# lucanest/Phyloformer

Hardware: AMD Instinct MI355X
Metric: alignments/sec, 60-leaf/500-site LG+GC-like MSAs, Phyloformer forward (pf.ckpt) (higher is better)
Workload: dtype f16x3-split MFMA (two fp16 limbs per operand, 3 passes), fp32 accumulate/residual

## Files before the change

phyloformer_amd/csrc/pf_device.hip.h:

```cpp
#pragma once
#include <hip/hip_runtime.h>
#include <stdint.h>

#include "pf_layout.h"

namespace pfk {

typedef float f32x4 __attribute__((ext_vector_type(4)));
typedef float f32x16 __attribute__((ext_vector_type(16)));
#if PF_F16
typedef _Float16 h16_t;
#define PF_MFMA(a, b, c) __builtin_amdgcn_mfma_f32_32x32x16_f16((a), (b), (c), 0, 0, 0)
#define PF_DOT2C "v_dot2c_f32_f16"
#define PF_CVT_PK "v_cvt_pk_f16_f32"
#define PF_NEG1_LO 0x0000bc00u
#define PF_NEG1_HI 0xbc000000u
#else
typedef __bf16 h16_t;
#define PF_MFMA(a, b, c) __builtin_amdgcn_mfma_f32_32x32x16_bf16((a), (b), (c), 0, 0, 0)
#define PF_DOT2C "v_dot2c_f32_bf16"
#define PF_CVT_PK "v_cvt_pk_bf16_f32"
#define PF_NEG1_LO 0x0000bf80u
#define PF_NEG1_HI 0xbf800000u
#endif
// ... 289 lines not shown
    const frag_t* wv_lo;
    const float* table;
    const uint8_t* idx;
    const int16_t* pair_i;
    const int16_t* pair_j;
    int B, N, P, Lloc;
    int flat;
    int nt_aln;
    int slots_aln;
    size_t trash_tok;
    int store_x_last;
    unsigned long long* prof;
    int ablate;
    float* sitemap;
    const float* w;
};

enum { MODE_FIRST = 0, MODE_MID = 1, MODE_LAST = 2, MODE_MID0 = 3, MODE_LAST_FOLD = 4 };

struct TilePos { int b, kt, r0, l0; };
template <bool FLAT>
__device__ __forceinline__ TilePos tile_pos(const MainArgs& a, int task, int ntiles) {
    TilePos q;
    q.b = task / a.nt_aln;
    q.kt = task - q.b * a.nt_aln;
    if (FLAT) { const int tok0 = q.kt * 32; q.r0 = tok0 / a.Lloc; q.l0 = tok0 - q.r0 * a.Lloc; }
    else { q.r0 = q.kt / ntiles; q.l0 = (q.kt - q.r0 * ntiles) * 32; }
    return q;
}
template <bool FLAT>
__device__ __forceinline__ TilePos tile_next(const MainArgs& a, TilePos q) {
    if (++q.kt == a.nt_aln) { q.b++; q.kt = 0; q.r0 = 0; q.l0 = 0; return q; }
    q.l0 += 32;
// ... 2 lines not shown
}
struct LanePos { size_t tok0; int toff, l, nvalid, wrap; bool valid, in_r1; };
template <bool FLAT>
__device__ __forceinline__ LanePos lane_pos(const MainArgs& a, const TilePos& q, int t) {
    LanePos o;
    o.tok0 = ((size_t)q.b * a.P + q.r0) * a.Lloc + q.l0;
    const int left = FLAT ? a.P * a.Lloc - q.kt * 32 : a.Lloc - q.l0;
    o.nvalid = min(32, left);
    o.wrap = (FLAT && q.r0 + 1 < a.P) ? min(32, a.Lloc - q.l0) : 32;
    o.valid = t < o.nvalid;
    o.toff = min(t, o.nvalid - 1);
    o.in_r1 = o.toff >= o.wrap;
    o.l = q.l0 + o.toff - (o.in_r1 ? a.Lloc : 0);
    return o;
}
__device__ __forceinline__ void part_range(int flat, int pr, int nparts, int P, int L, int slots_aln, long* first, int* count) {
    if (!flat) { *first = (long)pr * nparts; *count = nparts; return; }
    const int b = pr / P, p = pr - b * P;
    const int k0 = (int)(((long)p * L) >> 5), k1 = (int)((((long)p + 1) * L - 1) >> 5);
    *first = (long)b * slots_aln + k0 + p;
    *count = k1 - k0 + 1;
}

template <int LO, int HI>
__device__ __forceinline__ void image_to_lds(const frag_t* src, unsigned char* smem) {
    static_assert(LO % 64 == 0 && HI % 64 == 0, "the image is copied in whole waves");
    const int wv = threadIdx.x >> 6, ln = threadIdx.x & 63;
#pragma unroll
    for (int k = 0; k < (HI - LO + MAIN_THREADS - 1) / MAIN_THREADS; ++k) {
        const int f0 = LO + k * MAIN_THREADS + wv * 64;
        if (f0 < HI) __builtin_amdgcn_global_load_lds(src + f0 + ln, smem + (size_t)f0 * 16, 16, 0, 0);
    }
}

template <int MODE, bool FLAT, bool SITEMAP = false, bool WEIGHTED = false>
__global__ void __launch_bounds__(MAIN_THREADS, MAIN_WAVES / 4) k_main(MainArgs a) {
    constexpr bool LAST = MODE == MODE_LAST || MODE == MODE_LAST_FOLD;
    constexpr bool FOLD = MODE == MODE_LAST_FOLD;
    static_assert(!SITEMAP || LAST, "the site map is the head's: last block only");
    static_assert(!WEIGHTED || (!SITEMAP && MODE != MODE_FIRST), "weighted launches: blocks' own modes, no site map");
    extern __shared__ __attribute__((aligned(16))) unsigned char smem[];
    lds_frag_t lw = (lds_frag_t)smem;
    lds_f32_t lc = (lds_f32_t)(smem + FRAG_END * 16);

    {
        const float cv = a.consts[min((int)threadIdx.x, CONST_LEN - 1)];
        if (FOLD) {
            image_to_lds<FRAG_W1, FRAG_W2>(a.wimg, smem);
            image_to_lds<FRAG_WO, FRAG_U + U_FRAGS>(a.wimg, smem);
        } else {
            image_to_lds<(MODE == MODE_FIRST) ? FRAG_WV : 0, LAST ? FRAG_WV : FRAG_END>(a.wimg, smem);
        }
        static_assert(CONST_LEN <= MAIN_THREADS, "one constant per thread");
// ... 23 lines not shown

    {
        const int nwaves = gridDim.x * MAIN_WAVES;
#ifndef PF_RUN_MAX
#define PF_RUN_MAX 8
#endif
        const int run = max(1, min(PF_RUN_MAX, ntasks / (nwaves * 8)));
        int run0 = (blockIdx.x * MAIN_WAVES + wave) * run;
        const int task0 = run0, task1 = ntasks;
        TilePos cur = tile_pos<FLAT>(a, min(task0, ntasks - 1), ntiles);
        int frag_row = -1;
        frag_t mfr[4];
        f32x4 rqv = {0.f, 0.f, 0.f, 0.f};
        f32x4 px[8], pctx[8], pqr, pqc;
        int pri = 0, prj = 0;
        auto prefetch = [&](const TilePos& np) {
            const LanePos nl = lane_pos<FLAT>(a, np, t);
            const int ll = nl.l, pb = np.b;
            const size_t tk = nl.tok0 + nl.toff;
            if (MODE == MODE_MID0) {
                const uint8_t* ib = a.idx + (size_t)pb * a.N * a.Lloc + ll;
                const int pp = np.r0 + (nl.in_r1 ? 1 : 0);
                pri = residue(ib[(size_t)a.pair_i[pp] * a.Lloc]);
                prj = residue(ib[(size_t)a.pair_j[pp] * a.Lloc]);
            } else {
                const f32x4* xp = reinterpret_cast<const f32x4*>(a.x + tk * 64 + 4 * h);
#pragma unroll
                for (int g = 0; g < 8; ++g) px[g] = xp[2 * g];
            }
            pqr = *reinterpret_cast<const f32x4*>(a.qrow + tk * 4);
            pqc = *reinterpret_cast<const f32x4*>(a.qcol + tk * 4);
            if (MODE != MODE_FIRST) {
                int hq = h;
                asm volatile("" : "+v"(hq));
                const f32x4* cp = reinterpret_cast<const f32x4*>(a.ctx + ((size_t)pb * a.Lloc + ll) * 64 + 4 * hq);
#pragma unroll
                for (int g = 0; g < 8; ++g) pctx[g] = cp[2 * g];
            }
        };
        if (MODE != MODE_FIRST && task0 < task1) prefetch(cur);

        for (int task = task0; task < task1;) {
            const int b = cur.b;
            const int row = b * a.P + cur.r0;
            int ntask = task + 1;
            TilePos nxt = tile_next<FLAT>(a, cur);
            if (ntask == run0 + run) {
                run0 += nwaves * run;
                ntask = run0;
                if (ntask < task1) nxt = tile_pos<FLAT>(a, ntask, ntiles);
            }
            const LanePos lp = lane_pos<FLAT>(a, cur, t);
            const bool straddle = lp.wrap < 32;
            int ai = 0, aj = 0;
            if (MODE == MODE_FIRST) { const int pp = cur.r0 + (lp.in_r1 ? 1 : 0); ai = a.pair_i[pp]; aj = a.pair_j[pp]; }
            auto load_mfr = [&](int r) {
                const frag_t* mf = a.mfrag + (size_t)r * 128 + t;
#pragma unroll
                for (int q = 0; q < 4; ++q) mfr[q] = mf[q * 32];
                typedef const f32x4 __attribute__((address_space(4)))* const_f32x4_t;
                rqv = *(const_f32x4_t)(unsigned long long)(a.rq + (size_t)__builtin_amdgcn_readfirstlane(r) * 4);
                frag_row = r;
            };
            if (MODE != MODE_FIRST && row != frag_row) load_mfr(row);
            const bool valid = lp.valid;
// ... 4 lines not shown
            float wt = 1.f;
            if (WEIGHTED && LAST) wt = a.w[(size_t)b * a.Lloc + lc_];

            if (MODE == MODE_FIRST) {
                const int ri = residue(a.idx[((size_t)b * a.N + ai) * a.Lloc + lc_]);
                const int rj = residue(a.idx[((size_t)b * a.N + aj) * a.Lloc + lc_]);
                const f32x4* ti = reinterpret_cast<const f32x4*>(a.table + ri * 64 + 4 * h);
                const f32x4* tj = reinterpret_cast<const f32x4*>(a.table + rj * 64 + 4 * h);
#pragma unroll
                for (int g = 0; g < 8; ++g) {
                    f32x4 u = ti[2 * g], w = tj[2 * g];
#pragma unroll
                    for (int i = 0; i < 4; ++i) x[4 * g + i] = u[i] + w[i];
                }
            } else {
                if (MODE == MODE_MID0) {
                    const f32x4* ti = reinterpret_cast<const f32x4*>(a.table + pri * 64 + 4 * h);
                    const f32x4* tj = reinterpret_cast<const f32x4*>(a.table + prj * 64 + 4 * h);
#pragma unroll
                    for (int g = 0; g < 8; ++g) {
                        const f32x4 u = ti[2 * g], w = tj[2 * g];
#pragma unroll
                        for (int i = 0; i < 4; ++i) x[4 * g + i] = u[i] + w[i];
                    }
                } else {
#pragma unroll
                    for (int g = 0; g < 8; ++g)
#pragma unroll
                        for (int i = 0; i < 4; ++i) x[4 * g + i] = px[g][i];
                }
                PF_TICK(0);
// ... 89 lines not shown
                    }
                    PF_TICK(3);
                } else if (!(a.ablate & 16)) {
                    frag_t xb_hi[4], xb_lo[4];
                    {
                        float xn[32];
                        ln_pair(x, xn);
#pragma unroll
                        for (int s = 0; s < 4; ++s) split8(&xn[8 * s], xb_hi[s], xb_lo[s]);
                    }
                    f32x16 oa[2];
                    load_acc_bias(oa[0], lch + CONST_B2);
                    load_acc_bias(oa[1], lch + CONST_B2 + 32);
#pragma unroll
                    for (int j = 0; j < 32; ++j) oa[j >> 4][j & 15] += x[j];
                    if (ntask < task1) prefetch(nxt);
                    PF_TICK(2);
#pragma unroll 1
                    for (int T = 0; T < 8; ++T) {
                        f32x16 ha;
                        lds_frag_t f1 = w1p + T * 512;
                        lds_frag_t f2 = w2p + T * 256;
                        lds_f32_t bp = lch + CONST_B1 + 32 * T;
                        PF_OPAQUE(f1); PF_OPAQUE(f2); PF_OPAQUE(bp);
                        load_acc_bias(ha, bp);
                        frag_t fh = f1[0], fl = f1[64];
#pragma unroll
                        for (int s = 0; s < 4; ++s) {
                            frag_t nh, nl;
                            if (s < 3) { nh = f1[(s + 1) * 128]; nl = f1[(s + 1) * 128 + 64]; }
                            else { nh = f2[0]; nl = f2[64]; }
// ... 218 lines not shown
                if (valid) {
                    if (WEIGHTED) {
                        acc += wl * s;
                        acce += wl * e;
                    } else {
                        acc += s;
                        acce += e;
                    }
                    const size_t tok = row0 + l;
                    if (a.x) {
                        const int ra = rr / 22, rb = rr - 22 * ra;
                        const f32x4 xa = *reinterpret_cast<const f32x4*>(emb + ra * 64 + 4 * cl);
                        const f32x4 xb = *reinterpret_cast<const f32x4*>(emb + rb * 64 + 4 * cl);
                        *reinterpret_cast<f32x4*>(a.x + tok * 64 + 4 * cl) = xa + xb;
                    }
                    if (cl == 0) *reinterpret_cast<f32x4*>(a.qrow + tok * 4) = e;
                }
            };
            if (lbase + 64 <= a.Lloc) {
#pragma unroll 4
                for (int it = 0; it < 16; ++it) site(it, true);
            } else {
                for (int it = 0; it < nit; ++it) site(it, lbase + 4 * it + sg < a.Lloc);
            }
            cur = nxt;
            wcur = wnxt;
        }
#pragma unroll
        for (int i = 0; i < 4; ++i) {
            acc[i] += __shfl_xor(acc[i], 16);
            acc[i] += __shfl_xor(acc[i], 32);
// ... 147 lines not shown
    const float* x;
    const float* qrow;
    const float* mrow;
    float* qcol;
    float* part;
    const float* wqk;
    const float* bqk;
    const float* brow;
    int B, P, Lloc, G, nchunks;
    int sub, S, fine;
    const float* table;
    const uint8_t* idx;
    const int16_t* pair_i;
    const int16_t* pair_j;
    int N;
};
constexpr int CPART = 4 * 64 + 8;

constexpr int CS_SLOT = 2 * 256 + 64;
#ifndef PF_CS_RING
#define PF_CS_RING 4
#endif
#ifndef PF_CS_MT
#define PF_CS_MT 16
#endif
template <bool EMBED, int RING, int MT>
#ifndef PF_CS_WAVES
#define PF_CS_WAVES 2
#endif
__global__ void __launch_bounds__(256, PF_CS_WAVES) k_colstats(ColStatsArgs a) {
    static_assert(!(EMBED && RING), "block 0 reads residue bytes, not x");
    static_assert(RING % 2 == 0, "pairs are consumed two at a time");
    static_assert(MT == 16 || MT == 8, "pair matrices are staged 16 or 8 at a time (runs are multiples of 8)");
    constexpr int LDS_MST = 2 * MT * MROW, LDS_RING = RING ? 4 * RING * CS_SLOT : 0, LDS_EMB = EMBED ? 22 * 64 : 0;
    constexpr int PIJ_CAP = 640;
    __shared__ __attribute__((aligned(16))) float lds_all[LDS_MST + LDS_RING + LDS_EMB + (EMBED ? PIJ_CAP : 0)];
    float* const mst = lds_all;
    float* const xring = lds_all + LDS_MST;
    float* const emb = lds_all + LDS_MST + LDS_RING;
    int16_t* const pij = reinterpret_cast<int16_t*>(lds_all + LDS_MST + LDS_RING + LDS_EMB);
    if (EMBED) {
        constexpr int NV = 22 * 64 / 4;
        const f32x4* tsrc = reinterpret_cast<const f32x4*>(a.table);
        const int i0 = threadIdx.x, i1 = threadIdx.x + 256;
        static_assert(NV <= 2 * 256, "two vectors per thread cover the table");
        const f32x4 v0 = tsrc[min(i0, NV - 1)], v1 = tsrc[min(i1, NV - 1)];
        if (i0 < NV) reinterpret_cast<f32x4*>(emb)[i0] = v0;
        if (i1 < NV) reinterpret_cast<f32x4*>(emb)[i1] = v1;
    }
    const int lane = threadIdx.x & 63, wave = threadIdx.x >> 6;
    const int ts = lane >> 3, cl = lane & 7;
    const int per = (a.P + a.G - 1) / a.G;

    f32x2 w2[4][8];
#pragma unroll
    for (int o = 0; o < 8; o += 2)
#pragma unroll
        for (int q = 0; q < 2; ++q) {
            const f32x4 u0 = *reinterpret_cast<const f32x4*>(a.wqk + o * 64 + 8 * cl + 4 * q);
            const f32x4 u1 = *reinterpret_cast<const f32x4*>(a.wqk + (o + 1) * 64 + 8 * cl + 4 * q);
#pragma unroll
            for (int i = 0; i < 4; ++i) w2[o >> 1][4 * q + i] = f32x2{u0[i], u1[i]};
        }
// ... 32 lines not shown

    f32x4 nx0[2], nx1[2], nqr[2];
    int nri[2] = {0, 0}, nrj[2] = {0, 0};
    const bool pij_lds = EMBED && (p1 - p0) <= PIJ_CAP;
    if (pij_lds) {
        for (int i = threadIdx.x; i < p1 - p0; i += 256) { pij[i] = a.pair_i[p0 + i]; pij[PIJ_CAP + i] = a.pair_j[p0 + i]; }
        __syncthreads();
    }
    auto fetch = [&](int p, int u) {
        const int pc = min(p, a.P - 1);
        const size_t tk = ((size_t)b * a.P + pc) * a.Lloc + lcl;
        if (!EMBED) {
            nx0[u] = *reinterpret_cast<const f32x4*>(a.x + tk * 64 + 8 * cl);
            nx1[u] = *reinterpret_cast<const f32x4*>(a.x + tk * 64 + 8 * cl + 4);
        }
        nqr[u] = *reinterpret_cast<const f32x4*>(a.qrow + tk * 4);
    };
    float* const wring = xring + (RING ? wave * RING * CS_SLOT : 0);
    const int lq = min(chunk * 32 + wave * 8 + ((lane & 31) >> 2), a.Lloc - 1);
    auto issue = [&](int p, size_t lane_off) {
        const int pc = min(p, a.P - 1);
        const size_t row = ((size_t)b * a.P + pc) * a.Lloc;
        float* dst = wring + ((p - p0) % RING) * CS_SLOT;
        const float* xs = a.x + row * 64 + lane_off;
        __builtin_amdgcn_global_load_lds(xs, dst, 16, 0, 0);
        __builtin_amdgcn_global_load_lds(xs + 4, dst + 256, 16, 0, 0);
        __builtin_amdgcn_global_load_lds(a.qrow + (row + lq) * 4 + (lane & 3), dst + 512, 4, 0, 0);
    };
    const size_t lane_off0 = (size_t)lcl * 64 + 8 * cl;
    auto take = [&](int p, int u) {
        const float* slot = wring + ((p - p0) % RING) * CS_SLOT;
// ... 3 lines not shown
    };
    auto fetch_idx = [&](int p, int u) {
        const int pc = min(p, a.P - 1);
        const uint8_t* ib = a.idx + (size_t)b * a.N * a.Lloc + lcl;
        const int pl = min(pc, p1 - 1) - p0;
        const int si = pij_lds ? (int)pij[pl] : (int)a.pair_i[pc];
        const int sj = pij_lds ? (int)pij[PIJ_CAP + pl] : (int)a.pair_j[pc];
        nri[u] = residue(ib[(size_t)si * a.Lloc]);
        nrj[u] = residue(ib[(size_t)sj * a.Lloc]);
    };
    auto lookup = [&](int u) {
        const float* ei = emb + nri[u] * 64 + 8 * cl;
        const float* ej = emb + nrj[u] * 64 + 8 * cl;
        nx0[u] = *reinterpret_cast<const f32x4*>(ei) + *reinterpret_cast<const f32x4*>(ej);
        nx1[u] = *reinterpret_cast<const f32x4*>(ei + 4) + *reinterpret_cast<const f32x4*>(ej + 4);
    };
    auto stage = [&](int pt, int buf) {
        const f32x4* src = reinterpret_cast<const f32x4*>(a.mrow + ((size_t)b * a.P + pt) * MROW);
        const int n4 = min(MT, p1 - pt) * (MROW / 4);
        float* dst = mst + (size_t)buf * MT * MROW;
#pragma unroll
        for (int k = 0; k < MT * MROW / 4 / 256; ++k) {
            const int i = (int)threadIdx.x + 256 * k;
            __builtin_amdgcn_global_load_lds(src + min(i, n4 - 1), dst + (256 * k + 64 * wave) * 4, 16, 0, 0);
        }
    };
    stage(p0, 0);
    if (RING) {
#pragma unroll
        for (int i = 0; i < RING; ++i) issue(p0 + i, lane_off0);
// ... 262 lines not shown
```

phyloformer_amd/csrc/pf_host_prep.h:

```cpp
#pragma once
#include <algorithm>
#include <cmath>
#include <cstdint>
#include <cstring>
#include <vector>

#include "pf_layout.h"

namespace pfhost {
using namespace pfk;

inline uint16_t f2bf(float f) {
    uint32_t u;
    std::memcpy(&u, &f, 4);
    if ((u & 0x7fffffffu) > 0x7f800000u) return uint16_t((u >> 16) | 0x40);
    u += 0x7fffu + ((u >> 16) & 1u);
    return uint16_t(u >> 16);
}
inline float bf2f(uint16_t b) {
    uint32_t u = uint32_t(b) << 16;
    float f;
    std::memcpy(&f, &u, 4);
    return f;
}
// ... 180 lines not shown
                    zk += (double)r.wk[hh * E + c] * y;
                }
                q[hh] = elu1(zq);
                k[hh] = elu1(zk);
            }
            float* row = out.data() + (size_t)(a * NA + b) * PAIRTAB_W;
            for (int co = 0; co < E; ++co) {
                double v = 0;
                for (int c = 0; c < E; ++c) v += (double)r.wv[co * E + c] * (double)r.g[c] * xn[c];
                row[co] = (float)(k[co >> 4] * v);
            }
            for (int hh = 0; hh < NH; ++hh) { row[64 + hh] = (float)q[hh]; row[68 + hh] = (float)k[hh]; }
        }
}

struct TilePlan { int flat, nt_aln, slots_aln; };
inline TilePlan tile_plan_core(int P, int Lloc, int tile_force) {
    TilePlan t;
    const int ntiles = (Lloc + 31) / 32;
    const double waste = (double)(ntiles * 32 - Lloc) / (ntiles * 32), straddle = 0.10 * 32.0 / std::max(Lloc, 1);
    t.flat = (Lloc >= 32 && waste > straddle && tile_force != 0) ? 1 : 0;
    if (tile_force == 1 && Lloc >= 32 && Lloc % 32 != 0) t.flat = 1;
    t.nt_aln = t.flat ? (int)(((long)P * Lloc + 31) / 32) : P * ntiles;
    t.slots_aln = t.flat ? t.nt_aln + P : t.nt_aln;
    return t;
}

inline int colstats_groups(int , int P, int Lloc) {
    const int chunks = (Lloc + 31) / 32;
    int G = std::max((128 + chunks - 1) / chunks, (P + 639) / 640);
// ... 22 lines not shown
```

phyloformer_amd/csrc/pf_layout.h:

```cpp
#pragma once

#ifndef PF_F16
#define PF_F16 1
#endif

namespace pfk {

constexpr int E = 64;
constexpr int NH = 4;
constexpr int HD = 16;
constexpr int FF = 256;
constexpr int NA = 22;
constexpr int SROW = 72;
constexpr int MROW = 4 * 64;
constexpr float LN_EPS = 1e-5f;

constexpr int FRAG_W1 = 0;
constexpr int FRAG_W2 = FRAG_W1 + 8 * 4 * 2 * 64;
constexpr int FRAG_WO = FRAG_W2 + 2 * 16 * 2 * 64;
constexpr int FRAG_WV = FRAG_WO + 2 * 4 * 2 * 64;
constexpr int FRAG_QK = FRAG_WV + 2 * 4 * 64;
#ifndef PF_WVLO_LDS
#define PF_WVLO_LDS 4
#endif
// ... 2 lines not shown
constexpr int FRAG_END = FRAG_WVLO + WVLO_LDS * 64;
constexpr int FRAG_U = FRAG_WV;
constexpr int U_FRAGS = FF * 4 / 16;
static_assert(FRAG_U + U_FRAGS <= FRAG_END, "the folded head fits the last block's tail");
constexpr int WVLO_FRAGS = 2 * 4 * 64;
constexpr int CONST_B1 = 0, CONST_B2 = 256, CONST_BQK = 320, CONST_HW = 328, CONST_HB = 392,
              CONST_C0 = 393, CONST_BOC = 400;
constexpr int CONST_LEN = 464;
constexpr int MAIN_LDS_BYTES = FRAG_END * 16 + CONST_LEN * 4;
constexpr int MFRAG_PER_PAIR = 2 * 2 * 32;

constexpr int MAIN_THREADS = 512;
constexpr int MAIN_WAVES = MAIN_THREADS / 64;

constexpr int PAIRTAB_ROWS = 22 * 22, PAIRTAB_W = 72;

}
```

phyloformer_amd/csrc/pf_lib.hip:

```cpp
#include <hip/hip_runtime.h>
#include <dlfcn.h>

#include <algorithm>
#include <cmath>
#include <cstdarg>
#include <cstdio>
#include <cstdlib>
#include <cstring>
#include <functional>
#include <map>
#include <mutex>
#include <string>
#include <type_traits>
#include <vector>

#include "../../include/phyloformer_amd.h"
#include "pf_device.hip.h"
#include "pf_mha.hip.h"
#include "pf_precise.hip.h"
#include "pf_generic.hip.h"
#include "pf_boot.hip.h"
#include "pf_sites.hip.h"
#include "pf_sitemap.hip.h"
#include "pf_sites_host.h"
// ... 131 lines not shown
    hipEvent_t ev_fork = nullptr, ev_join = nullptr;
    hipDeviceProp_t prop;
    std::string err;
    int64_t max_seqs = 200;
    bool profile = false;
    bool profile_main_only = false;
    bool debug_keep = false;
    int ablate = 0;
    unsigned long long* phase_prof = nullptr;
    bool phase_prof_last = false;
    bool head_fold = true;
    bool force_rccl = false;
    int64_t ws_limit_bytes = (int64_t)24 << 30;
    float* table = nullptr;
    float* pair_table = nullptr;
    bool embed_mfma = false;
    int colstats_fine = -1;
    bool colstats_ring = true;
    bool materialize_x0 = false;
    float* first_consts = nullptr;
    float* first_img = nullptr;
    std::vector<BlockDev> blk;
    std::vector<void*> owned;
    int pair_n = -1;
    int16_t* pair_i = nullptr;
    int16_t* pair_j = nullptr;
    size_t ws_bytes = 0;
    char* ws = nullptr;
    size_t ws2_bytes = 0;
    char* ws2 = nullptr;
// ... 120 lines not shown
    if ((uint64_t)view.len != blob_len)
        return fail(h, PF_EINVAL, "weight blob has %llu floats, expected %llu",
                    (unsigned long long)blob_len, (unsigned long long)view.len);
    std::vector<float> table((size_t)NA * E);
    build_embed_table(view, E, E, table.data());
    int rc = upload(h, table, &h->table);
    if (rc) return rc;

    const int nb = (int)view.ffn.size();
    h->blk.resize(nb);

    {
        std::vector<float> ptab;
        build_pair_table(table.data(), view.row[0], ptab);
        if ((rc = upload(h, ptab, &h->pair_table))) return rc;
    }
    F16Ranges ranges;
    std::vector<std::vector<float>> row_bqk(nb);
    std::vector<std::vector<uint16_t>> row_tail(nb);
    for (int k = 0; k < nb; ++k) {
        BlockDev& d = h->blk[k];
        const AttnHost& r = view.row[k];
        const AttnHost& c = view.col[k];
        std::vector<float> wq, bq, wk, bk, wv, bv;
        fold(r.wq, r.bq, r.g, r.b, NH, E, wq, bq);
        fold(r.wk, r.bk, r.g, r.b, NH, E, wk, bk);
        fold(r.wv, r.bv, r.g, r.b, E, E, wv, bv);
        f16_note_attn(wv, bv, r.wo, false, &ranges);
        for (float v : wq) ranges.wmax = std::max(ranges.wmax, std::fabs((double)v));
        for (float v : wk) ranges.wmax = std::max(ranges.wmax, std::fabs((double)v));
// ... 66 lines not shown
    std::vector<uint16_t> img0((size_t)FRAG_END * 8, 0);
    std::copy(row_tail[0].begin(), row_tail[0].end(), img0.begin() + (size_t)FRAG_WV * 8);
    check_f16_ranges(h, ranges);
    if ((rc = upload(h, img0, &h->first_img))) return rc;
    return upload(h, cst0, &h->first_consts);
}

int ensure_pairs(pf_handle* h, int N) {
    if (h->pair_n == N) return PF_OK;
    const int P = N * (N - 1) / 2;
    std::vector<int16_t> pi(P), pj(P);
    int k = 0;
    for (int i = 0; i < N; ++i)
        for (int j = i + 1; j < N; ++j) { pi[k] = (int16_t)i; pj[k] = (int16_t)j; ++k; }
    if (h->pair_i) { hipFree(h->pair_i); hipFree(h->pair_j); h->pair_i = h->pair_j = nullptr; }
    HIPCHK(h, hipMalloc((void**)&h->pair_i, P * sizeof(int16_t)));
    HIPCHK(h, hipMalloc((void**)&h->pair_j, P * sizeof(int16_t)));
    HIPCHK(h, hipMemcpyAsync(h->pair_i, pi.data(), P * sizeof(int16_t), hipMemcpyHostToDevice, h->stream));
    HIPCHK(h, hipMemcpyAsync(h->pair_j, pj.data(), P * sizeof(int16_t), hipMemcpyHostToDevice, h->stream));
    HIPCHK(h, hipStreamSynchronize(h->stream));
    h->pair_n = N;
    return PF_OK;
}

size_t align_up(size_t v, size_t a) { return (v + a - 1) / a * a; }

TilePlan tile_plan(const pf_handle* h, int P, int Lloc) { return tile_plan_core(P, Lloc, h->tile_force); }

struct Workspace {
    float *x, *qrow, *qcol, *srow, *mrow, *part, *ctx, *mfrag, *spart, *outpart, *rq;
    int G;
    int sub, S, fine;
// ... 133 lines not shown
    return PF_OK;
}

MainArgs main_args(pf_handle* h, const ShardRun& r) {
    MainArgs m{};
    m.x = r.w.x; m.qrow = r.w.qrow; m.qcol = r.w.qcol;
    m.mfrag = reinterpret_cast<const frag_t*>(r.w.mfrag); m.rq = r.w.rq; m.ctx = r.w.ctx; m.spart = r.w.spart;
    m.outpart = r.w.outpart; m.table = h->table; m.idx = r.d_idx; m.pair_i = h->pair_i; m.pair_j = h->pair_j;
    m.B = r.B; m.N = r.N; m.P = r.P; m.Lloc = r.Lloc;
    m.flat = r.tp.flat; m.nt_aln = r.tp.nt_aln; m.slots_aln = r.tp.slots_aln;
    m.store_x_last = h->debug_keep ? 1 : 0;
    m.trash_tok = (size_t)r.B * r.P * r.Lloc;
    m.ablate = h->ablate;
    m.prof = h->phase_prof_last ? nullptr : h->phase_prof;
    m.w = r.d_w;
    return m;
}

bool x0_on_the_fly(const pf_handle* h) {
    return !h->materialize_x0 && !h->embed_mfma && h->n_blocks > 1;
}

int phase_first(pf_handle* h, const ShardRun& r) {
    if (!r.Lloc) return zero_fill(h, r.w.srow, (size_t)r.B * r.P * SROW);
    int rc;
    if (h->embed_mfma) {
        MainArgs m = main_args(h, r);
        m.wimg = reinterpret_cast<const frag_t*>(h->first_img); m.consts = h->first_consts;
        m.wv_lo = reinterpret_cast<const frag_t*>(h->blk[0].wv_lo);
        rc = launch_main<MODE_FIRST>(h, m, K_EMBED);
        if (rc) return rc;
    } else {
        float* x0 = (x0_on_the_fly(h) && !h->debug_keep) ? nullptr : r.w.x;
        EmbedArgs e{r.d_idx, h->pair_i, h->pair_j, h->pair_table, h->table, x0, r.w.qrow, r.w.srow,
                    r.B, r.N, r.P, r.Lloc, h->bad_idx_dev, r.d_w};
        const int ntasks = r.B * r.P, wpb = EMBED_THREADS / 64;
        const int grid = std::max(1, std::min(h->prop.multiProcessorCount, (ntasks + wpb - 1) / wpb));
        ProfScope ps(h, K_EMBED);
        if (r.d_w) hipLaunchKernelGGL(k_embed<true>, dim3(grid), dim3(EMBED_THREADS), EMBED_LDS_BYTES, h->cur, e);
        else hipLaunchKernelGGL(k_embed<false>, dim3(grid), dim3(EMBED_THREADS), EMBED_LDS_BYTES, h->cur, e);
        HIPCHK(h, hipGetLastError());
    }
    if (h->debug_keep) return save_tap(h, "x0", r.w.x, (size_t)r.B * r.P * r.Lloc * 64);
    return PF_OK;
}

int tiles_of(int Lloc) { return (Lloc + 31) / 32; }

int launch_rowsum(pf_handle* h, const ShardRun& r, RowStats* rs) {
// ... 40 lines not shown
                     d.row_woT, d.row_bv, d.row_bo, d.col_bo,
                     B * P, rs.nparts, (float)r.L_total, rs.flat, P, Lloc, r.tp.slots_aln, 1};
        const int groups = (B * P + 3) / 4;
        a.iters = std::max(1, std::min(16, groups / (4 * 8 * std::max(1, h->prop.multiProcessorCount))));
        a.rq = w.rq;
        a.b_scale = 1.f;
        for (long lim = 16384; lim < (long)r.L_total && a.b_scale > 1.f / 256.f; lim *= 2) a.b_scale *= 0.5f;
        a.a_scale = 1.f / a.b_scale;
        a.wst = r.d_wst;
        ProfScope ps(h, K_ROWFIN);
        hipLaunchKernelGGL(k_rowfin, dim3((groups + a.iters - 1) / a.iters), dim3(256), 0, h->cur, a);
        HIPCHK(h, hipGetLastError());
    }
    {
        ColStatsArgs a{w.x, w.qrow, w.mrow, w.qcol, w.part, d.col_wqk, d.col_bqk, d.row_bo, B, P, Lloc, w.G, (Lloc + 31) / 32,
                       w.sub, w.S, w.fine, h->table, r.d_idx, h->pair_i, h->pair_j, r.N};
        ProfScope ps(h, K_COLSTATS);
        const unsigned nblk = (unsigned)(B * a.nchunks * w.nparts());
        if (k == 0 && x0_on_the_fly(h))
            hipLaunchKernelGGL((k_colstats<true, 0, 16>), dim3(nblk), dim3(256), 0, h->cur, a);
        else if (h->colstats_ring)
            hipLaunchKernelGGL((k_colstats<false, PF_CS_RING, PF_CS_MT>), dim3(nblk), dim3(256), 0, h->cur, a);
        else
            hipLaunchKernelGGL((k_colstats<false, 0, 16>), dim3(nblk), dim3(256), 0, h->cur, a);
        HIPCHK(h, hipGetLastError());
    }
    {
        ColFinArgs a{w.part, w.ctx, d.col_wvT, d.col_bv, B, Lloc, w.G, (float)P, P, w.sub, w.S, w.fine};
        ProfScope ps(h, K_COLFIN);
        hipLaunchKernelGGL(k_colfin, dim3(B * Lloc), dim3(COLFIN_THREADS), 0, h->cur, a);
        HIPCHK(h, hipGetLastError());
    }
    if (h->debug_keep) {
        if ((rc = save_tap(h, "ctx" + std::to_string(k), w.ctx, (size_t)B * Lloc * 64))) return rc;
        if ((rc = save_tap(h, "mrow" + std::to_string(k), w.mrow, (size_t)B * P * MROW))) return rc;
    }
    MainArgs m = main_args(h, r);
    m.wimg = reinterpret_cast<const frag_t*>(d.wimg);
    m.consts = d.consts;
    if (k + 1 < h->n_blocks) {
        m.wv_lo = reinterpret_cast<const frag_t*>(h->blk[k + 1].wv_lo);
        const bool first = k == 0 && x0_on_the_fly(h);
        if (r.d_w) rc = first ? launch_main<MODE_MID0, false, true>(h, m, K_MAIN) : launch_main<MODE_MID, false, true>(h, m, K_MAIN);
        else rc = first ? launch_main<MODE_MID0>(h, m, K_MAIN) : launch_main<MODE_MID>(h, m, K_MAIN);
        if (rc) return rc;
    } else {
        m.wv_lo = nullptr;
        if (h->phase_prof_last) m.prof = h->phase_prof;
        m.sitemap = r.d_smap;
        if (!h->head_fold) {
            if ((rc = r.d_w      ? launch_main<MODE_LAST, false, true>(h, m, K_MAIN)
                      : r.d_smap ? launch_main<MODE_LAST, true>(h, m, K_MAIN) : launch_main<MODE_LAST>(h, m, K_MAIN))) return rc;
        } else {
            if ((rc = r.d_w      ? launch_main<MODE_LAST_FOLD, false, true>(h, m, K_MAIN)
                      : r.d_smap ? launch_main<MODE_LAST_FOLD, true>(h, m, K_MAIN) : launch_main<MODE_LAST_FOLD>(h, m, K_MAIN)))
                return rc;
            if (h->debug_keep) {
                MainArgs md = m;
                md.outpart = w.spart;
// ... 1062 lines not shown
    return read_blob(nullptr, n_blocks, embed_dim, n_heads).len;
}

static int open_device(int device, pf_handle** out) {
    int ndev = 0;
    hipError_t e = hipGetDeviceCount(&ndev);
    if (e != hipSuccess || ndev == 0)
        return fail(nullptr, PF_EHIP, "no HIP device available (%s); there is no CPU fallback",
                    e != hipSuccess ? hipGetErrorString(e) : "device count is 0");
    if (device < 0 || device >= ndev) return fail(nullptr, PF_EINVAL, "device %d out of range (have %d)", device, ndev);
    pf_handle* h = new pf_handle();
    if (const char* e = getenv("PF_TWO_STREAMS")) h->two_streams = atoi(e) != 0;
    if (getenv("PF_ROW_TILES")) h->tile_force = 0;
    if (getenv("PF_FLAT_TILES")) h->tile_force = 1;
    if (const char* v = getenv("PF_COLSTATS_RING")) h->colstats_ring = atoi(v) != 0;
    h->device = device;
    int rc = PF_OK;
    do {
        if ((e = hipSetDevice(device)) != hipSuccess) { rc = fail(nullptr, PF_EHIP, "hipSetDevice: %s", hipGetErrorString(e)); break; }
        if ((e = hipGetDeviceProperties(&h->prop, device)) != hipSuccess) { rc = fail(nullptr, PF_EHIP, "hipGetDeviceProperties: %s", hipGetErrorString(e)); break; }
        if (std::string(h->prop.gcnArchName).rfind("gfx950", 0) != 0) {
            rc = fail(nullptr, PF_EHIP, "device %d is %s; this library is built for gfx950 only", device, h->prop.gcnArchName);
            break;
        }
        if ((e = hipStreamCreateWithFlags(&h->stream, hipStreamNonBlocking)) != hipSuccess) { rc = fail(nullptr, PF_EHIP, "hipStreamCreate: %s", hipGetErrorString(e)); break; }
        h->cur = h->stream;
        if ((e = hipHostMalloc((void**)&h->bad_idx_host, 3 * sizeof(unsigned), hipHostMallocMapped | hipHostMallocCoherent)) != hipSuccess ||
            (e = hipHostGetDevicePointer((void**)&h->bad_idx_dev, h->bad_idx_host, 0)) != hipSuccess) {
            rc = fail(nullptr, PF_EHIP, "hipHostMalloc (residue flag): %s", hipGetErrorString(e));
            break;
        }
        h->bad_idx_host[0] = h->bad_idx_host[1] = h->bad_idx_host[2] = 0u;
        const struct { const void* fn; int bytes; } big_lds[] = {
            {reinterpret_cast<const void*>(&k_main<MODE_FIRST, false>), MAIN_LDS_BYTES},
            {reinterpret_cast<const void*>(&k_main<MODE_MID, false>), MAIN_LDS_BYTES},
            {reinterpret_cast<const void*>(&k_main<MODE_MID0, false>), MAIN_LDS_BYTES},
            {reinterpret_cast<const void*>(&k_main<MODE_LAST, false>), MAIN_LDS_BYTES},
            {reinterpret_cast<const void*>(&k_main<MODE_LAST_FOLD, false>), MAIN_LDS_BYTES},
            {reinterpret_cast<const void*>(&k_main<MODE_FIRST, true>), MAIN_LDS_BYTES},
            {reinterpret_cast<const void*>(&k_main<MODE_MID, true>), MAIN_LDS_BYTES},
            {reinterpret_cast<const void*>(&k_main<MODE_MID0, true>), MAIN_LDS_BYTES},
            {reinterpret_cast<const void*>(&k_main<MODE_LAST, true>), MAIN_LDS_BYTES},
            {reinterpret_cast<const void*>(&k_main<MODE_LAST_FOLD, true>), MAIN_LDS_BYTES},
            {reinterpret_cast<const void*>(&k_main<MODE_LAST, false, true>), MAIN_LDS_BYTES},
            {reinterpret_cast<const void*>(&k_main<MODE_LAST_FOLD, false, true>), MAIN_LDS_BYTES},
            {reinterpret_cast<const void*>(&k_main<MODE_LAST, true, true>), MAIN_LDS_BYTES},
            {reinterpret_cast<const void*>(&k_main<MODE_LAST_FOLD, true, true>), MAIN_LDS_BYTES},
            {reinterpret_cast<const void*>(&k_main<MODE_MID, false, false, true>), MAIN_LDS_BYTES},
            {reinterpret_cast<const void*>(&k_main<MODE_MID0, false, false, true>), MAIN_LDS_BYTES},
            {reinterpret_cast<const void*>(&k_main<MODE_LAST, false, false, true>), MAIN_LDS_BYTES},
            {reinterpret_cast<const void*>(&k_main<MODE_LAST_FOLD, false, false, true>), MAIN_LDS_BYTES},
            {reinterpret_cast<const void*>(&k_main<MODE_MID, true, false, true>), MAIN_LDS_BYTES},
            {reinterpret_cast<const void*>(&k_main<MODE_MID0, true, false, true>), MAIN_LDS_BYTES},
            {reinterpret_cast<const void*>(&k_main<MODE_LAST, true, false, true>), MAIN_LDS_BYTES},
            {reinterpret_cast<const void*>(&k_main<MODE_LAST_FOLD, true, false, true>), MAIN_LDS_BYTES},
            {reinterpret_cast<const void*>(&k_embed<false>), EMBED_LDS_BYTES},
            {reinterpret_cast<const void*>(&k_embed<true>), EMBED_LDS_BYTES},
        };
        for (const auto& k : big_lds)
            if ((e = hipFuncSetAttribute(k.fn, hipFuncAttributeMaxDynamicSharedMemorySize, k.bytes)) != hipSuccess) {
                rc = fail(nullptr, PF_EHIP, "hipFuncSetAttribute: %s", hipGetErrorString(e));
                break;
            }
        if (rc) break;
    } while (0);
    if (rc) { pf_destroy(h); return rc; }
    *out = h;
    return PF_OK;
// ... 77 lines not shown
    delete h;
    return PF_OK;
}

const char* pf_last_error(const pf_handle_t* h) { return h ? h->err.c_str() : g_create_error.c_str(); }

int pf_set_option(pf_handle_t* h, const char* key, int64_t value) {
    if (!h || !key) return PF_EINVAL;
    const std::string k(key);
    if (k == "max_seqs") h->max_seqs = value;
    else if (k == "profile") { drain_profile(h); h->profile = value != 0; h->profile_main_only = value == 2; }
    else if (k == "debug_keep") h->debug_keep = value != 0;
    else if (k == "embed_mfma") h->embed_mfma = value != 0;
    else if (k == "colstats_fine") h->colstats_fine = value < 0 ? -1 : (value != 0);
    else if (k == "materialize_x0") h->materialize_x0 = value != 0;
    else if (k == "overlap") h->overlap = value != 0;
    else if (k == "two_streams") h->two_streams = value != 0;
    else if (k == "reserve_cus") h->reserve_cus = (int)std::max<int64_t>(0, std::min<int64_t>(value, 128));
    else if (k == "ablate") h->ablate = (int)value;
    else if (k == "head_fold") h->head_fold = value != 0;
    else if (k == "force_rccl") h->force_rccl = value != 0;
    else if (k == "colstats_ring") h->colstats_ring = value != 0;
    else if (k == "precise") h->precise = value < 0 ? -1 : (value != 0);
    else if (k == "recheck_above") h->recheck_above = value > 0 ? (double)value : 0.0;
    else if (k == "precise_ffn_valu") h->precise_ffn_valu = value != 0;
    else if (k == "generic") {
        if (h->arch_generic && !value)
            return fail(h, PF_EINVAL, "embed_dim %d / n_heads %d runs on the generic kernels only (option generic cannot be 0)",
                        h->garch.E, h->garch.NH);
        h->generic = value != 0;
// ... 639 lines not shown
```

Measured before the change: 556.6.

## Read block-0 embeddings and row queries from a residue-pair class table

```diff
diff --git a/phyloformer_amd/csrc/pf_device.hip.h b/phyloformer_amd/csrc/pf_device.hip.h
--- a/phyloformer_amd/csrc/pf_device.hip.h
+++ b/phyloformer_amd/csrc/pf_device.hip.h
@@ -327,9 +327,10 @@
     int ablate;
     float* sitemap;
     const float* w;
+    const float* ctab;
 };
 
-enum { MODE_FIRST = 0, MODE_MID = 1, MODE_LAST = 2, MODE_MID0 = 3, MODE_LAST_FOLD = 4 };
+enum { MODE_FIRST = 0, MODE_MID = 1, MODE_LAST = 2, MODE_MID0 = 3, MODE_LAST_FOLD = 4, MODE_MID0_GATHER = 5 };
 
 struct TilePos { int b, kt, r0, l0; };
 template <bool FLAT>
@@ -362,6 +363,13 @@
     o.l = q.l0 + o.toff - (o.in_r1 ? a.Lloc : 0);
     return o;
 }
+__device__ __forceinline__ int pair_seq_uniform(const int16_t* tab, int row) {
+    typedef const int __attribute__((address_space(4)))* const_i32_t;
+    const int r = __builtin_amdgcn_readfirstlane(row);
+    const int w = *(const_i32_t)(unsigned long long)(reinterpret_cast<const int*>(tab) + (r >> 1));
+    return (r & 1) ? (w >> 16) : (w & 0xffff);
+}
+
 __device__ __forceinline__ void part_range(int flat, int pr, int nparts, int P, int L, int slots_aln, long* first, int* count) {
     if (!flat) { *first = (long)pr * nparts; *count = nparts; return; }
     const int b = pr / P, p = pr - b * P;
@@ -385,6 +393,7 @@
 __global__ void __launch_bounds__(MAIN_THREADS, MAIN_WAVES / 4) k_main(MainArgs a) {
     constexpr bool LAST = MODE == MODE_LAST || MODE == MODE_LAST_FOLD;
     constexpr bool FOLD = MODE == MODE_LAST_FOLD;
+    constexpr bool CLASS0 = MODE == MODE_MID0, GATHER0 = MODE == MODE_MID0_GATHER;
     static_assert(!SITEMAP || LAST, "the site map is the head's: last block only");
     static_assert(!WEIGHTED || (!SITEMAP && MODE != MODE_FIRST), "weighted launches: blocks' own modes, no site map");
     extern __shared__ __attribute__((aligned(16))) unsigned char smem[];
@@ -438,21 +447,42 @@
         f32x4 rqv = {0.f, 0.f, 0.f, 0.f};
         f32x4 px[8], pctx[8], pqr, pqc;
         int pri = 0, prj = 0;
+        struct RowSeqs { int i0, j0, i1, j1; };
+        auto row_seqs = [&](const TilePos& np) {
+            RowSeqs s;
+            s.i0 = pair_seq_uniform(a.pair_i, np.r0);
+            s.j0 = pair_seq_uniform(a.pair_j, np.r0);
+            s.i1 = FLAT ? pair_seq_uniform(a.pair_i, min(np.r0 + 1, a.P - 1)) : s.i0;
+            s.j1 = FLAT ? pair_seq_uniform(a.pair_j, min(np.r0 + 1, a.P - 1)) : s.j0;
+            return s;
+        };
+        auto prefetch_res = [&](const TilePos& np, const RowSeqs& rs) {
+            const LanePos nl = lane_pos<FLAT>(a, np, t);
+            const uint8_t* ib = a.idx + (size_t)np.b * a.N * a.Lloc + nl.l;
+            pri = ib[(size_t)((FLAT && nl.in_r1) ? rs.i1 : rs.i0) * a.Lloc];
+            prj = ib[(size_t)((FLAT && nl.in_r1) ? rs.j1 : rs.j0) * a.Lloc];
+        };
         auto prefetch = [&](const TilePos& np) {
             const LanePos nl = lane_pos<FLAT>(a, np, t);
             const int ll = nl.l, pb = np.b;
             const size_t tk = nl.tok0 + nl.toff;
-            if (MODE == MODE_MID0) {
+            if (GATHER0) {
                 const uint8_t* ib = a.idx + (size_t)pb * a.N * a.Lloc + ll;
                 const int pp = np.r0 + (nl.in_r1 ? 1 : 0);
                 pri = residue(ib[(size_t)a.pair_i[pp] * a.Lloc]);
                 prj = residue(ib[(size_t)a.pair_j[pp] * a.Lloc]);
+            } else if (CLASS0) {
+                const float* cr = a.ctab + (residue(pri) * NA + residue(prj)) * CLASSTAB_W;
+                const f32x4* xp = reinterpret_cast<const f32x4*>(cr + 4 * h);
+#pragma unroll
+                for (int g = 0; g < 8; ++g) px[g] = xp[2 * g];
+                pqr = *reinterpret_cast<const f32x4*>(cr + E);
             } else {
                 const f32x4* xp = reinterpret_cast<const f32x4*>(a.x + tk * 64 + 4 * h);
 #pragma unroll
                 for (int g = 0; g < 8; ++g) px[g] = xp[2 * g];
             }
-            pqr = *reinterpret_cast<const f32x4*>(a.qrow + tk * 4);
+            if (!CLASS0) pqr = *reinterpret_cast<const f32x4*>(a.qrow + tk * 4);
             pqc = *reinterpret_cast<const f32x4*>(a.qcol + tk * 4);
             if (MODE != MODE_FIRST) {
                 int hq = h;
@@ -462,7 +492,22 @@
                 for (int g = 0; g < 8; ++g) pctx[g] = cp[2 * g];
             }
         };
-        if (MODE != MODE_FIRST && task0 < task1) prefetch(cur);
+        auto tile_after = [&](int tk, int r0, TilePos& pos) {
+            int nt = tk + 1;
+            TilePos n = tile_next<FLAT>(a, pos);
+            if (nt == r0 + run) {
+                nt = r0 + nwaves * run;
+                if (nt < task1) n = tile_pos<FLAT>(a, nt, ntiles);
+            }
+            pos = n;
+            return nt;
+        };
+        if (CLASS0 && task0 < task1) {
+            prefetch_res(cur, row_seqs(cur));
+            prefetch(cur);
+            TilePos n1 = cur;
+            if (tile_after(task0, run0, n1) < task1) prefetch_res(n1, row_seqs(n1));
+        } else if (MODE != MODE_FIRST && task0 < task1) prefetch(cur);
 
         for (int task = task0; task < task1;) {
             const int b = cur.b;
@@ -473,6 +518,13 @@
                 run0 += nwaves * run;
                 ntask = run0;
                 if (ntask < task1) nxt = tile_pos<FLAT>(a, ntask, ntiles);
+            }
+            int ntask2 = ntask;
+            TilePos nx2 = nxt;
+            RowSeqs rs2 = {0, 0, 0, 0};
+            if (CLASS0 && ntask < task1) {
+                ntask2 = tile_after(ntask, run0, nx2);
+                if (ntask2 < task1) rs2 = row_seqs(nx2);
             }
             const LanePos lp = lane_pos<FLAT>(a, cur, t);
             const bool straddle = lp.wrap < 32;
@@ -507,7 +559,7 @@
                     for (int i = 0; i < 4; ++i) x[4 * g + i] = u[i] + w[i];
                 }
             } else {
-                if (MODE == MODE_MID0) {
+                if (GATHER0) {
                     const f32x4* ti = reinterpret_cast<const f32x4*>(a.table + pri * 64 + 4 * h);
                     const f32x4* tj = reinterpret_cast<const f32x4*>(a.table + prj * 64 + 4 * h);
 #pragma unroll
@@ -627,7 +679,10 @@
                     load_acc_bias(oa[1], lch + CONST_B2 + 32);
 #pragma unroll
                     for (int j = 0; j < 32; ++j) oa[j >> 4][j & 15] += x[j];
-                    if (ntask < task1) prefetch(nxt);
+                    if (ntask < task1) {
+                        prefetch(nxt);
+                        if (CLASS0 && ntask2 < task1) prefetch_res(nx2, rs2);
+                    }
                     PF_TICK(2);
 #pragma unroll 1
                     for (int T = 0; T < 8; ++T) {
@@ -876,7 +931,7 @@
                         const f32x4 xb = *reinterpret_cast<const f32x4*>(emb + rb * 64 + 4 * cl);
                         *reinterpret_cast<f32x4*>(a.x + tok * 64 + 4 * cl) = xa + xb;
                     }
-                    if (cl == 0) *reinterpret_cast<f32x4*>(a.qrow + tok * 4) = e;
+                    if (a.qrow && cl == 0) *reinterpret_cast<f32x4*>(a.qrow + tok * 4) = e;
                 }
             };
             if (lbase + 64 <= a.Lloc) {
@@ -1054,6 +1109,7 @@
     const int16_t* pair_i;
     const int16_t* pair_j;
     int N;
+    const float* ctab;
 };
 constexpr int CPART = 4 * 64 + 8;
 
@@ -1064,21 +1120,24 @@
 #ifndef PF_CS_MT
 #define PF_CS_MT 16
 #endif
-template <bool EMBED, int RING, int MT>
+template <bool EMBED, int RING, int MT, bool QCLASS = false>
 #ifndef PF_CS_WAVES
 #define PF_CS_WAVES 2
 #endif
 __global__ void __launch_bounds__(256, PF_CS_WAVES) k_colstats(ColStatsArgs a) {
     static_assert(!(EMBED && RING), "block 0 reads residue bytes, not x");
+    static_assert(EMBED || !QCLASS, "residue classes are block 0's");
     static_assert(RING % 2 == 0, "pairs are consumed two at a time");
     static_assert(MT == 16 || MT == 8, "pair matrices are staged 16 or 8 at a time (runs are multiples of 8)");
     constexpr int LDS_MST = 2 * MT * MROW, LDS_RING = RING ? 4 * RING * CS_SLOT : 0, LDS_EMB = EMBED ? 22 * 64 : 0;
+    constexpr int LDS_QT = QCLASS ? PAIRTAB_ROWS * 4 : 0;
     constexpr int PIJ_CAP = 640;
-    __shared__ __attribute__((aligned(16))) float lds_all[LDS_MST + LDS_RING + LDS_EMB + (EMBED ? PIJ_CAP : 0)];
+    __shared__ __attribute__((aligned(16))) float lds_all[LDS_MST + LDS_RING + LDS_EMB + LDS_QT + (EMBED ? PIJ_CAP : 0)];
     float* const mst = lds_all;
     float* const xring = lds_all + LDS_MST;
     float* const emb = lds_all + LDS_MST + LDS_RING;
-    int16_t* const pij = reinterpret_cast<int16_t*>(lds_all + LDS_MST + LDS_RING + LDS_EMB);
+    float* const qtab = lds_all + LDS_MST + LDS_RING + LDS_EMB;
+    int16_t* const pij = reinterpret_cast<int16_t*>(lds_all + LDS_MST + LDS_RING + LDS_EMB + LDS_QT);
     if (EMBED) {
         constexpr int NV = 22 * 64 / 4;
         const f32x4* tsrc = reinterpret_cast<const f32x4*>(a.table);
@@ -1087,6 +1146,13 @@
         const f32x4 v0 = tsrc[min(i0, NV - 1)], v1 = tsrc[min(i1, NV - 1)];
         if (i0 < NV) reinterpret_cast<f32x4*>(emb)[i0] = v0;
         if (i1 < NV) reinterpret_cast<f32x4*>(emb)[i1] = v1;
+        if (QCLASS) {
+            static_assert(PAIRTAB_ROWS <= 2 * 256, "two class rows per thread cover the table");
+            const f32x4 q0 = *reinterpret_cast<const f32x4*>(a.ctab + (size_t)min(i0, PAIRTAB_ROWS - 1) * CLASSTAB_W + E);
+            const f32x4 q1 = *reinterpret_cast<const f32x4*>(a.ctab + (size_t)min(i1, PAIRTAB_ROWS - 1) * CLASSTAB_W + E);
+            if (i0 < PAIRTAB_ROWS) reinterpret_cast<f32x4*>(qtab)[i0] = q0;
+            if (i1 < PAIRTAB_ROWS) reinterpret_cast<f32x4*>(qtab)[i1] = q1;
+        }
     }
     const int lane = threadIdx.x & 63, wave = threadIdx.x >> 6;
     const int ts = lane >> 3, cl = lane & 7;
@@ -1149,7 +1215,7 @@
             nx0[u] = *reinterpret_cast<const f32x4*>(a.x + tk * 64 + 8 * cl);
             nx1[u] = *reinterpret_cast<const f32x4*>(a.x + tk * 64 + 8 * cl + 4);
         }
-        nqr[u] = *reinterpret_cast<const f32x4*>(a.qrow + tk * 4);
+        if (!QCLASS) nqr[u] = *reinterpret_cast<const f32x4*>(a.qrow + tk * 4);
     };
     float* const wring = xring + (RING ? wave * RING * CS_SLOT : 0);
     const int lq = min(chunk * 32 + wave * 8 + ((lane & 31) >> 2), a.Lloc - 1);
@@ -1183,6 +1249,7 @@
         const float* ej = emb + nrj[u] * 64 + 8 * cl;
         nx0[u] = *reinterpret_cast<const f32x4*>(ei) + *reinterpret_cast<const f32x4*>(ej);
         nx1[u] = *reinterpret_cast<const f32x4*>(ei + 4) + *reinterpret_cast<const f32x4*>(ej + 4);
+        if (QCLASS) nqr[u] = *reinterpret_cast<const f32x4*>(qtab + (nri[u] * NA + nrj[u]) * 4);
     };
     auto stage = [&](int pt, int buf) {
         const f32x4* src = reinterpret_cast<const f32x4*>(a.mrow + ((size_t)b * a.P + pt) * MROW);
diff --git a/phyloformer_amd/csrc/pf_host_prep.h b/phyloformer_amd/csrc/pf_host_prep.h
--- a/phyloformer_amd/csrc/pf_host_prep.h
+++ b/phyloformer_amd/csrc/pf_host_prep.h
@@ -218,6 +218,20 @@
         }
 }
 
+inline void build_class_table(const float* table, const std::vector<float>& ptab, std::vector<float>& out) {
+    out.assign((size_t)PAIRTAB_ROWS * CLASSTAB_W, 0.f);
+    for (int a = 0; a < NA; ++a)
+        for (int b = 0; b < NA; ++b) {
+            const int c = a * NA + b;
+            float* row = out.data() + (size_t)c * CLASSTAB_W;
+            for (int ch = 0; ch < E; ++ch) {
+                volatile float s = table[a * E + ch] + table[b * E + ch];
+                row[ch] = s;
+            }
+            for (int hh = 0; hh < NH; ++hh) row[E + hh] = ptab[(size_t)c * PAIRTAB_W + 64 + hh];
+        }
+}
+
 struct TilePlan { int flat, nt_aln, slots_aln; };
 inline TilePlan tile_plan_core(int P, int Lloc, int tile_force) {
     TilePlan t;
diff --git a/phyloformer_amd/csrc/pf_layout.h b/phyloformer_amd/csrc/pf_layout.h
--- a/phyloformer_amd/csrc/pf_layout.h
+++ b/phyloformer_amd/csrc/pf_layout.h
@@ -40,5 +40,6 @@
 constexpr int MAIN_WAVES = MAIN_THREADS / 64;
 
 constexpr int PAIRTAB_ROWS = 22 * 22, PAIRTAB_W = 72;
+constexpr int CLASSTAB_W = 68;
 
 }
diff --git a/phyloformer_amd/csrc/pf_lib.hip b/phyloformer_amd/csrc/pf_lib.hip
--- a/phyloformer_amd/csrc/pf_lib.hip
+++ b/phyloformer_amd/csrc/pf_lib.hip
@@ -169,6 +169,8 @@
     int64_t ws_limit_bytes = (int64_t)24 << 30;
     float* table = nullptr;
     float* pair_table = nullptr;
+    float* class_table = nullptr;
+    int block0_classes = 1;
     bool embed_mfma = false;
     int colstats_fine = -1;
     bool colstats_ring = true;
@@ -319,6 +321,9 @@
         std::vector<float> ptab;
         build_pair_table(table.data(), view.row[0], ptab);
         if ((rc = upload(h, ptab, &h->pair_table))) return rc;
+        std::vector<float> ctab;
+        build_class_table(table.data(), ptab, ctab);
+        if ((rc = upload(h, ctab, &h->class_table))) return rc;
     }
     F16Ranges ranges;
     std::vector<std::vector<float>> row_bqk(nb);
@@ -415,8 +420,8 @@
     for (int i = 0; i < N; ++i)
         for (int j = i + 1; j < N; ++j) { pi[k] = (int16_t)i; pj[k] = (int16_t)j; ++k; }
     if (h->pair_i) { hipFree(h->pair_i); hipFree(h->pair_j); h->pair_i = h->pair_j = nullptr; }
-    HIPCHK(h, hipMalloc((void**)&h->pair_i, P * sizeof(int16_t)));
-    HIPCHK(h, hipMalloc((void**)&h->pair_j, P * sizeof(int16_t)));
+    HIPCHK(h, hipMalloc((void**)&h->pair_i, (P + 1) * sizeof(int16_t)));
+    HIPCHK(h, hipMalloc((void**)&h->pair_j, (P + 1) * sizeof(int16_t)));
     HIPCHK(h, hipMemcpyAsync(h->pair_i, pi.data(), P * sizeof(int16_t), hipMemcpyHostToDevice, h->stream));
     HIPCHK(h, hipMemcpyAsync(h->pair_j, pj.data(), P * sizeof(int16_t), hipMemcpyHostToDevice, h->stream));
     HIPCHK(h, hipStreamSynchronize(h->stream));
@@ -580,12 +585,15 @@
     m.ablate = h->ablate;
     m.prof = h->phase_prof_last ? nullptr : h->phase_prof;
     m.w = r.d_w;
+    m.ctab = h->class_table;
     return m;
 }
 
 bool x0_on_the_fly(const pf_handle* h) {
     return !h->materialize_x0 && !h->embed_mfma && h->n_blocks > 1;
 }
+bool main_classes(const pf_handle* h) { return x0_on_the_fly(h) && h->block0_classes != 0; }
+bool colstats_classes(const pf_handle* h) { return x0_on_the_fly(h) && h->block0_classes == 1; }
 
 int phase_first(pf_handle* h, const ShardRun& r) {
     if (!r.Lloc) return zero_fill(h, r.w.srow, (size_t)r.B * r.P * SROW);
@@ -598,7 +606,8 @@
         if (rc) return rc;
     } else {
         float* x0 = (x0_on_the_fly(h) && !h->debug_keep) ? nullptr : r.w.x;
-        EmbedArgs e{r.d_idx, h->pair_i, h->pair_j, h->pair_table, h->table, x0, r.w.qrow, r.w.srow,
+        float* q0 = (main_classes(h) && colstats_classes(h) && !h->debug_keep) ? nullptr : r.w.qrow;
+        EmbedArgs e{r.d_idx, h->pair_i, h->pair_j, h->pair_table, h->table, x0, q0, r.w.srow,
                     r.B, r.N, r.P, r.Lloc, h->bad_idx_dev, r.d_w};
         const int ntasks = r.B * r.P, wpb = EMBED_THREADS / 64;
         const int grid = std::max(1, std::min(h->prop.multiProcessorCount, (ntasks + wpb - 1) / wpb));
@@ -669,10 +678,12 @@
     }
     {
         ColStatsArgs a{w.x, w.qrow, w.mrow, w.qcol, w.part, d.col_wqk, d.col_bqk, d.row_bo, B, P, Lloc, w.G, (Lloc + 31) / 32,
-                       w.sub, w.S, w.fine, h->table, r.d_idx, h->pair_i, h->pair_j, r.N};
+                       w.sub, w.S, w.fine, h->table, r.d_idx, h->pair_i, h->pair_j, r.N, h->class_table};
         ProfScope ps(h, K_COLSTATS);
         const unsigned nblk = (unsigned)(B * a.nchunks * w.nparts());
-        if (k == 0 && x0_on_the_fly(h))
+        if (k == 0 && colstats_classes(h))
+            hipLaunchKernelGGL((k_colstats<true, 0, 16, true>), dim3(nblk), dim3(256), 0, h->cur, a);
+        else if (k == 0 && x0_on_the_fly(h))
             hipLaunchKernelGGL((k_colstats<true, 0, 16>), dim3(nblk), dim3(256), 0, h->cur, a);
         else if (h->colstats_ring)
             hipLaunchKernelGGL((k_colstats<false, PF_CS_RING, PF_CS_MT>), dim3(nblk), dim3(256), 0, h->cur, a);
@@ -695,9 +706,11 @@
     m.consts = d.consts;
     if (k + 1 < h->n_blocks) {
         m.wv_lo = reinterpret_cast<const frag_t*>(h->blk[k + 1].wv_lo);
-        const bool first = k == 0 && x0_on_the_fly(h);
-        if (r.d_w) rc = first ? launch_main<MODE_MID0, false, true>(h, m, K_MAIN) : launch_main<MODE_MID, false, true>(h, m, K_MAIN);
-        else rc = first ? launch_main<MODE_MID0>(h, m, K_MAIN) : launch_main<MODE_MID>(h, m, K_MAIN);
+        const bool first = k == 0 && x0_on_the_fly(h), classes = first && main_classes(h);
+        if (r.d_w) rc = classes ? launch_main<MODE_MID0, false, true>(h, m, K_MAIN)
+                      : first   ? launch_main<MODE_MID0_GATHER, false, true>(h, m, K_MAIN) : launch_main<MODE_MID, false, true>(h, m, K_MAIN);
+        else rc = classes ? launch_main<MODE_MID0>(h, m, K_MAIN)
+                : first   ? launch_main<MODE_MID0_GATHER>(h, m, K_MAIN) : launch_main<MODE_MID>(h, m, K_MAIN);
         if (rc) return rc;
     } else {
         m.wv_lo = nullptr;
@@ -1790,6 +1803,7 @@
     if (getenv("PF_ROW_TILES")) h->tile_force = 0;
     if (getenv("PF_FLAT_TILES")) h->tile_force = 1;
     if (const char* v = getenv("PF_COLSTATS_RING")) h->colstats_ring = atoi(v) != 0;
+    if (const char* v = getenv("PF_BLOCK0_CLASSES")) h->block0_classes = (atoi(v) == 0 || atoi(v) == 2) ? atoi(v) : 1;
     h->device = device;
     int rc = PF_OK;
     do {
@@ -1811,11 +1825,13 @@
             {reinterpret_cast<const void*>(&k_main<MODE_FIRST, false>), MAIN_LDS_BYTES},
             {reinterpret_cast<const void*>(&k_main<MODE_MID, false>), MAIN_LDS_BYTES},
             {reinterpret_cast<const void*>(&k_main<MODE_MID0, false>), MAIN_LDS_BYTES},
+            {reinterpret_cast<const void*>(&k_main<MODE_MID0_GATHER, false>), MAIN_LDS_BYTES},
             {reinterpret_cast<const void*>(&k_main<MODE_LAST, false>), MAIN_LDS_BYTES},
             {reinterpret_cast<const void*>(&k_main<MODE_LAST_FOLD, false>), MAIN_LDS_BYTES},
             {reinterpret_cast<const void*>(&k_main<MODE_FIRST, true>), MAIN_LDS_BYTES},
             {reinterpret_cast<const void*>(&k_main<MODE_MID, true>), MAIN_LDS_BYTES},
             {reinterpret_cast<const void*>(&k_main<MODE_MID0, true>), MAIN_LDS_BYTES},
+            {reinterpret_cast<const void*>(&k_main<MODE_MID0_GATHER, true>), MAIN_LDS_BYTES},
             {reinterpret_cast<const void*>(&k_main<MODE_LAST, true>), MAIN_LDS_BYTES},
             {reinterpret_cast<const void*>(&k_main<MODE_LAST_FOLD, true>), MAIN_LDS_BYTES},
             {reinterpret_cast<const void*>(&k_main<MODE_LAST, false, true>), MAIN_LDS_BYTES},
@@ -1824,10 +1840,12 @@
             {reinterpret_cast<const void*>(&k_main<MODE_LAST_FOLD, true, true>), MAIN_LDS_BYTES},
             {reinterpret_cast<const void*>(&k_main<MODE_MID, false, false, true>), MAIN_LDS_BYTES},
             {reinterpret_cast<const void*>(&k_main<MODE_MID0, false, false, true>), MAIN_LDS_BYTES},
+            {reinterpret_cast<const void*>(&k_main<MODE_MID0_GATHER, false, false, true>), MAIN_LDS_BYTES},
             {reinterpret_cast<const void*>(&k_main<MODE_LAST, false, false, true>), MAIN_LDS_BYTES},
             {reinterpret_cast<const void*>(&k_main<MODE_LAST_FOLD, false, false, true>), MAIN_LDS_BYTES},
             {reinterpret_cast<const void*>(&k_main<MODE_MID, true, false, true>), MAIN_LDS_BYTES},
             {reinterpret_cast<const void*>(&k_main<MODE_MID0, true, false, true>), MAIN_LDS_BYTES},
+            {reinterpret_cast<const void*>(&k_main<MODE_MID0_GATHER, true, false, true>), MAIN_LDS_BYTES},
             {reinterpret_cast<const void*>(&k_main<MODE_LAST, true, false, true>), MAIN_LDS_BYTES},
             {reinterpret_cast<const void*>(&k_main<MODE_LAST_FOLD, true, false, true>), MAIN_LDS_BYTES},
             {reinterpret_cast<const void*>(&k_embed<false>), EMBED_LDS_BYTES},
@@ -1935,6 +1953,7 @@
     else if (k == "embed_mfma") h->embed_mfma = value != 0;
     else if (k == "colstats_fine") h->colstats_fine = value < 0 ? -1 : (value != 0);
     else if (k == "materialize_x0") h->materialize_x0 = value != 0;
+    else if (k == "block0_classes") h->block0_classes = (value == 0 || value == 2) ? (int)value : 1;
     else if (k == "overlap") h->overlap = value != 0;
     else if (k == "two_streams") h->two_streams = value != 0;
     else if (k == "reserve_cus") h->reserve_cus = (int)std::max<int64_t>(0, std::min<int64_t>(value, 128));
```

Result: no change. 559.2, median of 6 (+0.5%).
